# goodmattg/ndivplanning

Hardware: AMD Instinct MI355X
Metric: gan_train_steps_per_sec_traj8_batch64 (higher is better)
Workload: dtype f32; 1 GPU; BASELINE configs[1]: train_gan.py step (D update + G update), codes mode, batch=64 trajectories per GPU, traj_len=8, num_sample=6, noise_dim=2; rows_per_gpu=2688, global_batch=64, parallelism=dp1, hip_graph=True, steps_per_graph_launch=16, repeats=1, gradient_exchange=none

## Files before the change

ndivplanning_amd/csrc/ndp_device.h:

```cpp
#pragma once
#include <hip/hip_runtime.h>
#include <stdint.h>

namespace ndp {

typedef float f32x4 __attribute__((ext_vector_type(4)));
typedef float f32x2 __attribute__((ext_vector_type(2)));
typedef uint32_t u32x4 __attribute__((ext_vector_type(4)));

constexpr int kThreads = 256;
constexpr int kWaves = 4;
constexpr float kLreluSlope = 0.01f;

enum Act { ACT_NONE = 0, ACT_RELU = 1, ACT_LRELU = 2 };

__device__ __forceinline__ int lds_ld(int width) { return width + 4; }

template <int ACT>
__device__ __forceinline__ float act_fwd(float v) {
  if (ACT == ACT_RELU) return v > 0.f ? v : 0.f;
  if (ACT == ACT_LRELU) return v > 0.f ? v : v * kLreluSlope;
  return v;
}

template <int ACT>
__device__ __forceinline__ float act_bwd(float h, float g) {
  if (ACT == ACT_RELU) return h > 0.f ? g : 0.f;
  if (ACT == ACT_LRELU) return h > 0.f ? g : g * kLreluSlope;
  return g;
}

__device__ __forceinline__ void pin_vmem() { __builtin_amdgcn_sched_barrier(0x0786); }
__device__ __forceinline__ void pin_vmem_lds() { __builtin_amdgcn_sched_barrier(0x0606); }

__device__ __forceinline__ f32x4 mfma16(float a, float b, f32x4 c) {
#ifdef NDP_EXP_NOMFMA
  c[0] += a * b;
  return c;
#else
  return __builtin_amdgcn_mfma_f32_16x16x4f32(a, b, c, 0, 0, 0);
#endif
}

__device__ __forceinline__ int fwd_pack_offset(int j, int k, int in, int out) {
  const int per_wave = out >> 2, nt = out >> 6, nit = in >> 4;
  const int wave = j / per_wave, n = (j % per_wave) >> 4, c = j & 15;
  const int t = k >> 4, q = (k & 15) >> 2, e = k & 3;
  return (((wave * nt + n) * nit + t) * 64 + 16 * q + c) * 4 + e;
}
__device__ __forceinline__ int dgrad_pack_offset(int j, int k, int in, int out) {
  const int v_ = in >> 6, nit = out >> 4;
  const int wave = k / (16 * v_), c = (k % (16 * v_)) / v_, v = k % v_;
  const int t = j >> 4, q = (j & 15) >> 2, s = j & 3;
  return (((wave * nit + t) * 64 + 16 * q + c) * 4 + s) * v_ + v;
}

template <class T>
__device__ __forceinline__ T load_kernargs() {
  typedef const __attribute__((address_space(4))) void* kptr_t;
  kptr_t kp = (kptr_t)__builtin_amdgcn_kernarg_segment_ptr();
  constexpr int LAST = (((int)sizeof(T) - 4) / 64) * 64;
  constexpr int O1 = 64 < LAST ? 64 : LAST, O2 = 128 < LAST ? 128 : LAST, O3 = 192 < LAST ? 192 : LAST,
                O4 = 256 < LAST ? 256 : LAST, O5 = 320 < LAST ? 320 : LAST, O6 = 384 < LAST ? 384 : LAST,
                O7 = 448 < LAST ? 448 : LAST;
  static_assert(sizeof(T) <= 576, "argument struct too large for the 8-line prefetch");
  uint32_t t0, t1, t2, t3, t4, t5, t6, t7;
  asm volatile(
      "s_load_dword %0, %8, 0x0\n\ts_load_dword %1, %8, %9\n\ts_load_dword %2, %8, %10\n\t"
      "s_load_dword %3, %8, %11\n\ts_load_dword %4, %8, %12\n\ts_load_dword %5, %8, %13\n\t"
      "s_load_dword %6, %8, %14\n\ts_load_dword %7, %8, %15\n\ts_waitcnt lgkmcnt(0)"
      : "=&s"(t0), "=&s"(t1), "=&s"(t2), "=&s"(t3), "=&s"(t4), "=&s"(t5), "=&s"(t6), "=&s"(t7)
      : "s"(kp), "i"(O1), "i"(O2), "i"(O3), "i"(O4), "i"(O5), "i"(O6), "i"(O7)
      : "memory");
  uint64_t v = (uint64_t)kp;
  asm volatile("" : "+s"(v) : "s"(t0 | t1 | t2 | t3 | t4 | t5 | t6 | t7));
  T out;
  __builtin_memcpy(&out, (kptr_t)v, sizeof(T));
  return out;
}

template <int WALIGN>
__device__ __forceinline__ f32x4 ldg4(const float* p) {
#ifdef NDP_EXP_NOLOAD
  const float v = (float)(reinterpret_cast<uintptr_t>(p) & 1023) * 1e-3f;
  return f32x4{v, v + 1.f, v + 2.f, v + 3.f};
#endif
  if (WALIGN >= 4) {
    return *reinterpret_cast<const f32x4*>(p);
  } else {
    f32x2 lo = *reinterpret_cast<const f32x2*>(p);
    f32x2 hi = *reinterpret_cast<const f32x2*>(p + 2);
    f32x4 r = {lo[0], lo[1], hi[0], hi[1]};
    return r;
  }
}

template <int IN, int OUT, int WALIGN, bool PACKED, int RING = 96>
struct FwdW {
  static constexpr int NT = OUT / 64;
  static constexpr int NIT = IN / 16;
  static constexpr int PF0 = RING / (4 * NT);
  static constexpr int PF = PF0 < NIT ? PF0 : NIT;
  f32x4 ring[PF][NT];
  f32x4 wtail[NT];
  float bias_r[NT];
  const float* wbase;
  int ldw;

  __device__ __forceinline__ f32x4 frag(int n, int t) const {
    if (PACKED) {
      const int wave = threadIdx.x >> 6;
      return ldg4<4>(wbase + (size_t)((wave * NT + n) * NIT + t) * 256);
    }
// ... 306 lines not shown
      g[1] = fmaf(d, w[1], g[1]);
      g[2] = fmaf(d, w[2], g[2]);
      g[3] = fmaf(d, w[3], g[3]);
    }
    f32x4* hp = reinterpret_cast<f32x4*>(H + row * ldh + k);
    f32x4 h = *hp;
    h[0] = act_bwd<ACT>(h[0], g[0]);
    h[1] = act_bwd<ACT>(h[1], g[1]);
    h[2] = act_bwd<ACT>(h[2], g[2]);
    h[3] = act_bwd<ACT>(h[3], g[3]);
    *hp = h;
  }
}

template <int RT, int OUT>
__device__ __forceinline__ void input_dgrad_code(const float* dY, int ldd, const float* __restrict__ W, int ldw,
                                                 float* __restrict__ dX, int64_t ldx, int64_t row0, int64_t m) {
  static_assert(OUT % 16 == 0, "input_dgrad_code shape");
  constexpr int NIT = OUT / 16;
  const int lane = threadIdx.x & 63, wave = threadIdx.x >> 6;
  const int c = lane & 15, q = lane >> 4;
  const float* wp = W + (size_t)(4 * q) * ldw + 64 * wave + c;
  const float* dp = dY + c * ldd + 4 * q;
  f32x4 acc[RT][4];
#pragma unroll
  for (int r = 0; r < RT; ++r)
#pragma unroll
    for (int n = 0; n < 4; ++n) acc[r][n] = f32x4{0.f, 0.f, 0.f, 0.f};
#pragma unroll
  for (int t = 0; t < NIT; ++t) {
    float bv[4][4];
#pragma unroll
    for (int s = 0; s < 4; ++s)
#pragma unroll
      for (int n = 0; n < 4; ++n) bv[s][n] = wp[(size_t)(16 * t + s) * ldw + 16 * n];
    f32x4 av[RT];
#pragma unroll
    for (int r = 0; r < RT; ++r) av[r] = *reinterpret_cast<const f32x4*>(dp + r * 16 * ldd + 16 * t);
#pragma unroll
    for (int s = 0; s < 4; ++s)
#pragma unroll
      for (int r = 0; r < RT; ++r)
#pragma unroll
        for (int n = 0; n < 4; ++n) acc[r][n] = mfma16(av[r][s], bv[s][n], acc[r][n]);
  }
#pragma unroll
  for (int r = 0; r < RT; ++r)
#pragma unroll
    for (int i = 0; i < 4; ++i) {
      const int64_t row = row0 + r * 16 + 4 * q + i;
      if (row < m) {
#pragma unroll
        for (int n = 0; n < 4; ++n) dX[row * ldx + 64 * wave + 16 * n + c] = acc[r][n][i];
      }
    }
}

__device__ __forceinline__ void stg4_wt(float* base, uint32_t off, f32x4 v) {
  const uint64_t ub = reinterpret_cast<uint64_t>(base);
  const uint32_t hi = (uint32_t)__builtin_amdgcn_readfirstlane((int)(ub >> 32));
  const uint32_t lo = (uint32_t)__builtin_amdgcn_readfirstlane((int)(uint32_t)ub);
  const uint64_t sb = ((uint64_t)hi << 32) | (uint64_t)lo;
  const __amdgpu_buffer_rsrc_t rsrc =
      __builtin_amdgcn_make_buffer_rsrc(reinterpret_cast<float*>(sb), 0, 0x7fffffff, 0x00020000);
  __builtin_amdgcn_raw_buffer_store_b128(__builtin_bit_cast(u32x4, v), rsrc, (int)(off * 4u), 0, 16 );
}

template <int RT, int W, bool WT = false>
__device__ __forceinline__ void store_tile(float* __restrict__ dst, size_t gld,
                                           const float* src, int ld) {
  constexpr int R = 16 * RT;
  constexpr int NV = R * W / 4;
#ifdef NDP_EXP_NOSTORE
  if (gld == 0x7fffffff)
#endif
  for (int idx = threadIdx.x; idx < NV; idx += kThreads) {
    const int row = idx / (W / 4), k = 4 * (idx % (W / 4));
    const f32x4 v = *reinterpret_cast<const f32x4*>(src + row * ld + k);
    if constexpr (WT) stg4_wt(dst, (uint32_t)(row * (int)gld + k), v);
    else *reinterpret_cast<f32x4*>(dst + (size_t)row * gld + k) = v;
  }
}

template <int RT, int W>
struct TileRegs {
  static constexpr int NV = 16 * RT * W / 4;
  static constexpr int N = (NV + kThreads - 1) / kThreads;
  f32x4 v[N];
  __device__ __forceinline__ void load(const float* __restrict__ src, size_t gld) {
#pragma unroll
    for (int u = 0; u < N; ++u) {
      int idx = threadIdx.x + u * kThreads;
      idx = idx < NV ? idx : NV - 1;
      const int row = idx / (W / 4), k = 4 * (idx % (W / 4));
      v[u] = ldg4<4>(src + (size_t)row * gld + k);
    }
  }
  __device__ __forceinline__ void store(float* dst, int ld) const {
#pragma unroll
    for (int u = 0; u < N; ++u) {
      const int idx = threadIdx.x + u * kThreads;
      if (idx < NV) {
        const int row = idx / (W / 4), k = 4 * (idx % (W / 4));
        *reinterpret_cast<f32x4*>(dst + row * ld + k) = v[u];
      }
    }
  }
};

template <int RT, int W>
__device__ __forceinline__ void load_tile(float* dst, int ld,
                                          const float* __restrict__ src, size_t gld) {
  constexpr int R = 16 * RT;
  constexpr int NV = R * W / 4;
  for (int idx = threadIdx.x; idx < NV; idx += kThreads) {
    const int row = idx / (W / 4), k = 4 * (idx % (W / 4));
    *reinterpret_cast<f32x4*>(dst + row * ld + k) =
        *reinterpret_cast<const f32x4*>(src + (size_t)row * gld + k);
  }
}

template <int RT>
__device__ __forceinline__ void load_code_tile(float* dst, int ld,
                                               const float* __restrict__ code, int64_t ld_code,
                                               int rep, int64_t row0, int64_t m, bool vec4) {
  constexpr int R = 16 * RT;
  constexpr int NV = R * 64;
  for (int idx = threadIdx.x; idx < NV; idx += kThreads) {
    const int i = idx >> 6, k = 4 * (idx & 63);
    const int64_t row = row0 + i;
    f32x4 v = {0.f, 0.f, 0.f, 0.f};
    if (row < m) {
      const float* p = code + (row / rep) * ld_code + k;
      if (vec4) {
        v = *reinterpret_cast<const f32x4*>(p);
      } else {
        v[0] = p[0]; v[1] = p[1]; v[2] = p[2]; v[3] = p[3];
      }
    }
    *reinterpret_cast<f32x4*>(dst + i * ld + k) = v;
  }
}

__device__ __forceinline__ float wave_sum(float v) {
#pragma unroll
  for (int d = 32; d >= 1; d >>= 1) v += __shfl_xor(v, d, 64);
  return v;
}

__device__ __forceinline__ float block_sum(float v, float* red) {
  v = wave_sum(v);
  if ((threadIdx.x & 63) == 0) red[threadIdx.x >> 6] = v;
  __syncthreads();
  float r = 0.f;
  if (threadIdx.x == 0) {
    const int nw = blockDim.x >> 6;
    for (int w = 0; w < nw; ++w) r += red[w];
  }
  __syncthreads();
  return r;
}

}
```

ndivplanning_amd/csrc/ndp_kernels.hip:

```cpp
#include <hip/hip_runtime.h>
#include <math.h>
#include <stddef.h>
#include <stdint.h>

#include "ndp_device.h"

namespace ndp {

#ifdef NDP_STAMPS
__device__ unsigned long long* g_stamps = nullptr;
__device__ int g_stamp_kernel = 0;
#define NDP_STAMP_ON(id) (g_stamps != nullptr && (g_stamp_kernel == 0 || g_stamp_kernel == (id)))
#define NDP_STAMP_DECL __shared__ unsigned long long stamp_store_[64]; unsigned long long* stamp_lds_ = stamp_store_
#define NDP_STAMP_PTR stamp_lds_
#define NDP_STAMP(i)                                             \
  do {                                                           \
    if (threadIdx.x == 0) {                                      \
      stamp_lds_[2 * (i)] = clock64();                           \
      stamp_lds_[2 * (i) + 1] = wall_clock64();                  \
    }                                                            \
  } while (0)
#define NDP_STAMP_FLUSH(n, id)                                                              \
  do {                                                                                      \
    if (threadIdx.x == 0 && NDP_STAMP_ON(id))                                               \
// ... 435 lines not shown
  GNet net;
  int64_t m;
  const float *h1, *h2, *h3, *h4;
  const float* d_action;
  const float* d_action2;
  float *dy1, *dy2, *dy3, *dy4, *dy5;
};

constexpr int g_bwd_lds_floats() { return 16 * (132 + 68 + 132 + 260 + 4); }

template <bool PK>
__global__ __launch_bounds__(kThreads) void k_g_bwd(GBwdArgs a) {
  constexpr int R = 16;
  extern __shared__ __attribute__((aligned(16))) float smem[];
  float* H1 = smem;
  float* H2 = H1 + R * 132;
  float* H3 = H2 + R * 68;
  float* H4 = H3 + R * 132;
  float* DA = H4 + R * 260;
  const int64_t row0 = (int64_t)blockIdx.x * R;
  const GNet& n = a.net;

  DgW<128, 256, PK> g4;
  g4.preload(PK ? n.pg4 : n.w4, 128);
  load_tile<1, 128>(H1, 132, a.h1 + row0 * 128, 128);
  load_tile<1, 64>(H2, 68, a.h2 + row0 * 64, 64);
  load_tile<1, 128>(H3, 132, a.h3 + row0 * 128, 128);
  load_tile<1, 256>(H4, 260, a.h4 + row0 * 256, 256);
  if (threadIdx.x < R) {
    const int64_t row = row0 + threadIdx.x;
    f32x4 g = {0.f, 0.f, 0.f, 0.f};
    if (row < a.m) {
      g = *reinterpret_cast<const f32x4*>(a.d_action + row * 4);
      if (a.d_action2 != nullptr) g += *reinterpret_cast<const f32x4*>(a.d_action2 + row * 4);
    }
    *reinterpret_cast<f32x4*>(DA + threadIdx.x * 4) = g;
    *reinterpret_cast<f32x4*>(a.dy5 + row * 4) = g;
  }
  __syncthreads();
  layer_dgrad_narrow<1, 256, 4, ACT_RELU>(DA, 4, n.w5, H4, 260);
  __syncthreads();
  DgW<64, 128, PK> g3;
  g3.bind(PK ? n.pg3 : n.w3, 64);
  layer_dgrad_run<1, 128, 256, ACT_RELU, PK>(g4, H4, 260, H3, 132, g3);
  __syncthreads();
  DgW<128, 64, PK> g2;
  g2.bind(PK ? n.pg2 : n.w2, 128);
  layer_dgrad_run<1, 64, 128, ACT_RELU, PK>(g3, H3, 132, H2, 68, g2);
  __syncthreads();
  layer_dgrad_run<1, 128, 64, ACT_RELU, PK>(g2, H2, 68, H1, 132);
  __syncthreads();
  store_tile<1, 128>(a.dy1 + row0 * 128, 128, H1, 132);
  store_tile<1, 64>(a.dy2 + row0 * 64, 64, H2, 68);
  store_tile<1, 128>(a.dy3 + row0 * 128, 128, H3, 132);
  store_tile<1, 256>(a.dy4 + row0 * 256, 256, H4, 260);
}

struct GInGradArgs {
  const float* w1; int ld1, nz;
  const float* dy1;
  float* d_z; int64_t ld_dz;
  int64_t m;
};
__global__ __launch_bounds__(kThreads) void k_g_in_dgrad(GInGradArgs a) {
  constexpr int R = 16;
  __shared__ __attribute__((aligned(16))) float DY[R * 132];
  const int64_t row0 = (int64_t)blockIdx.x * R;
  load_tile<1, 128>(DY, 132, a.dy1 + row0 * 128, 128);
  __syncthreads();
  input_dgrad_code<1, 128>(DY, 132, a.w1, a.ld1, a.d_z, a.ld_dz, row0, a.m);
  const int i = threadIdx.x >> 4, j = threadIdx.x & 15;
  const int64_t row = row0 + i;
  if (j < a.nz && row < a.m) {
    float s = 0.f;
#pragma unroll 8
    for (int o = 0; o < 128; ++o) s = fmaf(DY[i * 132 + o], a.w1[(size_t)o * a.ld1 + CODE + j], s);
    a.d_z[row * a.ld_dz + CODE + j] = s;
  }
}

template <int W, int NP>
__device__ __forceinline__ void store_segment_sums(const float* dY, int ld, float* __restrict__ out,
                                                   int64_t row0, int K, int S, int entries_padded,
                                                   int tile, int ntiles) {
  const int f0 = (int)(row0 / K);
  for (int idx = threadIdx.x; idx < S * W; idx += kThreads) {
    const int sgm = idx / W, col = idx - sgm * W;
    const int64_t lo64 = (int64_t)(f0 + sgm) * K, hi64 = lo64 + K;
    const int lo = (int)(lo64 > row0 ? lo64 - row0 : 0);
    const int hi = (int)(hi64 < row0 + 16 ? hi64 - row0 : 16);
    float acc = 0.f;
    for (int r = lo; r < hi; ++r) {
#pragma unroll
      for (int ps = 0; ps < NP; ++ps) acc += dY[(ps * 16 + r) * ld + col];
    }
    out[((size_t)tile * S + sgm) * W + col] = acc;
  }
  if (tile == ntiles - 1) {
    const int first = ntiles * S;
    for (int idx = threadIdx.x; idx < (entries_padded - first) * W; idx += kThreads) out[(size_t)first * W + idx] = 0.f;
  }
}

struct PhaseAArgs {
  GNet g; DNet d;
  const float* code; int code_rep;
  const float* noise;
  float* noise_out; uint64_t noise_seed; const int32_t* noise_step;
  const float* actions;
  int64_t m, mpad;
  int64_t flat, rpad;
  float inv_m;
  float real_scale;
  float *gh1, *gh2, *gh3, *gh4;
  float* action_hat;
  float *h1, *h2, *h3, *dy1, *dy2, *dy3, *dl, *xa;
  float* loss_partials;
  float* dy1seg; int seg_s, seg_entries;
};

constexpr int kSW5 = 1024 + 8, kSW4 = 256 + 8;
constexpr int phase_a_lds_floats() {
  return 16 * (260 + TAILLD + 132 + 68 + 2) + 16 * 260 + 16 * 4 + 8 + kSW5 + kSW4;
}

template <int OUT, int NR>
__device__ __forceinline__ void code_rows_dot(const float* __restrict__ Wpacked, const float* code, float* part) {
  constexpr int PARTS = kThreads / OUT, SEG = CODE / PARTS;
  const int o = threadIdx.x % OUT, p = threadIdx.x / OUT;
  const float* w = Wpacked + fwd_pack_offset(o, p * SEG, CODE, OUT);
  const float* cr = code + p * SEG;
  float s0[NR], s1[NR];
#pragma unroll
  for (int j = 0; j < NR; ++j) s0[j] = s1[j] = 0.f;
#pragma unroll 2
  for (int t = 0; t < SEG / 16; ++t) {
#pragma unroll
    for (int q = 0; q < 4; ++q) {
      const f32x4 wv = *reinterpret_cast<const f32x4*>(w + t * 256 + q * 64);
#pragma unroll
      for (int j = 0; j < NR; ++j) {
        const f32x4 cv = *reinterpret_cast<const f32x4*>(cr + j * 260 + 16 * t + 4 * q);
        s0[j] = fmaf(wv[0], cv[0], s0[j]); s1[j] = fmaf(wv[1], cv[1], s1[j]);
        s0[j] = fmaf(wv[2], cv[2], s0[j]); s1[j] = fmaf(wv[3], cv[3], s1[j]);
      }
    }
  }
#pragma unroll
  for (int j = 0; j < NR; ++j) part[(j * PARTS + p) * OUT + o] = s0[j] + s1[j];
}
template <int NR>
__device__ __forceinline__ void load_code_rows(float* XC, const float* __restrict__ code, int64_t f0, int64_t nflat) {
  const int j = threadIdx.x >> 6, c4 = threadIdx.x & 63;
  if (j < NR) {
    f32x4 v = {0.f, 0.f, 0.f, 0.f};
    if (f0 + j < nflat) v = *reinterpret_cast<const f32x4*>(code + (size_t)(f0 + j) * CODE + 4 * c4);
    *reinterpret_cast<f32x4*>(XC + j * 260 + 4 * c4) = v;
  }
}
template <int OUT, int ACT, int NR>
__device__ __forceinline__ void fc1_from_code_rows(const float* part, const float* __restrict__ bias,
                                                   const float* __restrict__ Wt, int ldw, int ntail,
                                                   const float* XT, float* Y, int ldy, int rem0, int K) {
  constexpr int PARTS = kThreads / OUT, RSTEP = kThreads / OUT;
  const int o = threadIdx.x % OUT, r0 = threadIdx.x / OUT;
  float wt[16];
#pragma unroll
  for (int j = 0; j < 16; ++j) wt[j] = j < ntail ? Wt[(size_t)o * ldw + j] : 0.f;
  float base[NR];
#pragma unroll
  for (int j = 0; j < NR; ++j) {
    base[j] = bias[o];
#pragma unroll
    for (int p = 0; p < PARTS; ++p) base[j] += part[(j * PARTS + p) * OUT + o];
  }
  for (int r = r0; r < 16; r += RSTEP) {
    float s = base[0];
    if (NR > 1) {
      const int x = rem0 + r;
      const int idx = (x >= K) + (x >= 2 * K) + (x >= 3 * K);
#pragma unroll
      for (int j = 1; j < NR; ++j) s = idx >= j ? base[j] : s;
    }
#pragma unroll
    for (int j = 0; j < 16; ++j)
      if (j < ntail) s = fmaf(XT[r * TAILLD + j], wt[j], s);
    Y[r * ldy + o] = act_fwd<ACT>(s);
  }
}

constexpr bool kWtTilesCu1 = true;
constexpr bool kWtTilesLargeM = false;
constexpr bool kWtSlabs = true;
constexpr bool kWtSlabsWide = false;
constexpr bool wt_tiles(int RG) { return RG >= 96 ? kWtTilesCu1 : kWtTilesLargeM; }

template <bool PK, int RG, int NR>
__device__ __forceinline__ void phase_a_d_part(const PhaseAArgs& a, bool real, int tile, int ntiles,
                                               FwdW<256, 64, 4, PK, RG>& dw1, FwdW<64, 128, 4, PK, RG>& dw2, const float* cpd,
                                               float* XC, float* XT, float* B1,
                                               float* B2, float* L, float* DL, const float* W4S,
                                               unsigned long long* stamp_lds_) {
  constexpr int R = 16;
  constexpr bool WT = wt_tiles(RG);
  const DNet& d = a.d;
  (void)stamp_lds_;
  const int64_t row0 = (int64_t)tile * R;
  const int64_t nvalid = real ? a.flat : a.m;
  const int64_t g0 = (real ? 0 : a.rpad) + row0;
  NDP_STAMP(10);
  if (NR > 0) {
    fc1_from_code_rows<64, ACT_LRELU, (NR > 0 ? NR : 1)>(cpd, d.b1, d.w1, 260, ADIM, XT, B2, 68,
                                                         (int)(row0 % a.code_rep), a.code_rep);
  } else {
    dw2.bind(PK ? d.pf2 : d.w2, 64, d.b2, nullptr, 0);
    layer_fwd_run<1, 256, 64, ACT_LRELU, 4, PK>(dw1, XC, 260, B2, 68, XT, TAILLD, dw2);
  }
  NDP_STAMP(11);
  __syncthreads();
  NDP_STAMP(3);
  FwdW<128, 256, 4, PK, RG> dw3;
  dw3.bind(PK ? d.pf3 : d.w3, 128, d.b3, nullptr, 0);
  layer_fwd_run<1, 64, 128, ACT_LRELU, 4, PK>(dw2, B2, 68, B1, 132, nullptr, 0, dw3);
  __syncthreads();
  DgW<128, 256, PK, RG> dg3;
  dg3.bind(PK ? d.pg3 : d.w3, 128);
  layer_fwd_run<1, 128, 256, ACT_LRELU, 4, PK>(dw3, B1, 132, XC, 260, nullptr, 0, dg3);
  __syncthreads();
  NDP_STAMP(4);
  layer_fwd_narrow<1, 256, 1>(XC, 260, W4S, W4S + 256, L, 1);
  __syncthreads();
  float lsum = 0.f;
  if (threadIdx.x < R) {
    const int64_t row = row0 + threadIdx.x;
    const float target = real ? 1.f : 0.f;
    const float weight = real ? a.real_scale : 1.f;
    const float x = L[threadIdx.x];
    float dl = 0.f;
    if (row < nvalid) {
      lsum = weight * (fmaxf(x, 0.f) - x * target + log1pf(expf(-fabsf(x))));
      dl = weight * ((1.f / (1.f + expf(-x)) - target) * a.inv_m);
    }
    DL[threadIdx.x] = dl;
    a.dl[g0 + threadIdx.x] = dl;
  }
  if (threadIdx.x < 64) {
    const float tot = wave_sum(lsum);
    if (threadIdx.x == 0) a.loss_partials[blockIdx.x] = tot;
  }
  NDP_STAMP(5);
  store_tile<1, 64, WT>(a.h1 + g0 * 64, 64, B2, 68);
  store_tile<1, 128, WT>(a.h2 + g0 * 128, 128, B1, 132);
  store_tile<1, 256, WT>(a.h3 + g0 * 256, 256, XC, 260);
  if (threadIdx.x < R)
    if constexpr (WT) stg4_wt(a.xa + g0 * 4, 4 * threadIdx.x, *reinterpret_cast<const f32x4*>(XT + threadIdx.x * TAILLD));
    else *reinterpret_cast<f32x4*>(a.xa + (g0 + threadIdx.x) * 4) = *reinterpret_cast<const f32x4*>(XT + threadIdx.x * TAILLD);
  __syncthreads();
  NDP_STAMP(6);
  layer_dgrad_narrow<1, 256, 1, ACT_LRELU>(DL, 1, W4S, XC, 260);
  __syncthreads();
  DgW<64, 128, PK, RG> dg2;
  dg2.bind(PK ? d.pg2 : d.w2, 64);
  layer_dgrad_run<1, 128, 256, ACT_LRELU, PK>(dg3, XC, 260, B1, 132, dg2);
  __syncthreads();
  NDP_STAMP(7);
  layer_dgrad_run<1, 64, 128, ACT_LRELU, PK>(dg2, B1, 132, B2, 68);
  __syncthreads();
  if (real) store_tile<1, 64, WT>(a.dy1seg + ((size_t)a.seg_entries + row0) * 64, 64, B2, 68);
  else store_segment_sums<64, 1>(B2, 68, a.dy1seg, row0, a.code_rep, a.seg_s, a.seg_entries, tile, ntiles);
  store_tile<1, 64, WT>(a.dy1 + g0 * 64, 64, B2, 68);
  store_tile<1, 128, WT>(a.dy2 + g0 * 128, 128, B1, 132);
  store_tile<1, 256, WT>(a.dy3 + g0 * 256, 256, XC, 260);
}

constexpr int kPhaseASmallRing = 24;
template <bool PK, int RG, int NR>
__global__ __launch_bounds__(kThreads, (RG >= 96 ? 1 : 3)) void k_phase_a(PhaseAArgs a_segment) {
  constexpr bool DD = NR > 0;
  constexpr int NRR = NR > 0 ? NR : 1;
  constexpr bool WT = wt_tiles(RG);
  const PhaseAArgs a = RG >= 96 ? load_kernargs<PhaseAArgs>() : a_segment;
  constexpr int R = 16;
  extern __shared__ __attribute__((aligned(16))) float smem[];
  float* XC = smem;
  float* XT = XC + R * 260;
  float* B1 = XT + R * TAILLD;
  float* B2 = B1 + R * 132;
  float* B3 = B2 + R * 68;
  float* A = B3 + R * 260;
  float* L = A + R * 4;
  float* DL = L + R;
  float* red = DL + R;
  float* W5S = red + 8;
  float* W4S = W5S + kSW5;
  const int ntiles = (int)(a.mpad / R);
  const bool real = (int)blockIdx.x >= ntiles;
  const GNet& g = a.g;
  const DNet& d = a.d;
  NDP_STAMP_DECL;
  NDP_STAMP(0);

  FwdW<256, 64, 4, PK, RG> dw1;
  FwdW<64, 128, 4, PK, RG> dw2;
  if (!real) {
    const int tile = (int)blockIdx.x;
    const int64_t row0 = (int64_t)tile * R;
    FwdW<256, 128, 2, PK, RG> gw1;
    FwdW<128, 64, 4, PK, RG> gw2;
    f32x4 ct[R * 64 / kThreads];
    if (DD) {
      load_code_rows<NRR>(XC, a.code, (int64_t)((uint32_t)row0 / (uint32_t)a.code_rep), a.flat);
    } else {
#pragma unroll
      for (int u = 0; u < R * 64 / kThreads; ++u) {
        const int idx = threadIdx.x + u * kThreads;
        const int i = idx >> 6, k = 4 * (idx & 63);
        const int64_t row = row0 + i;
        const bool ok = row < a.m;
        const f32x4 v = *reinterpret_cast<const f32x4*>(a.code + (size_t)((uint32_t)(ok ? row : 0) / (uint32_t)a.code_rep) * CODE + k);
        ct[u] = ok ? v : f32x4{0.f, 0.f, 0.f, 0.f};
      }
    }
    const f32x4 w5r = *reinterpret_cast<const f32x4*>(g.w5 + 4 * threadIdx.x);
    const float b5r = g.b5[threadIdx.x & 3], w4r = d.w4[threadIdx.x], b4r = d.b4[0];
    float nv = 0.f;
    {
      static_assert(R * TAILLD == kThreads, "one noise element per thread");
      const int i = threadIdx.x / TAILLD, t = threadIdx.x % TAILLD;
      const int64_t row = row0 + i;
      if (row < a.m && t < g.nz) {
        if (a.noise_out != nullptr) {
          nv = philox_uniform((uint64_t)(row * g.nz + t), a.noise_seed, (uint32_t)*a.noise_step);
          a.noise_out[row * g.nz + t] = nv;
        } else {
          nv = a.noise[row * g.nz + t];
        }
      }
    }
    pin_vmem();
    if (DD) gw2.preload(PK ? g.pf2 : g.w2, 128, g.b2, nullptr, 0);
    else gw1.preload(PK ? g.pf1 : g.w1, g.ld1, g.b1, g.w1 + CODE, g.nz);
    NDP_STAMP(24);
    if (!DD) {
#pragma unroll
      for (int u = 0; u < R * 64 / kThreads; ++u) {
        const int idx = threadIdx.x + u * kThreads;
        *reinterpret_cast<f32x4*>(XC + (idx >> 6) * 260 + 4 * (idx & 63)) = ct[u];
      }
    }
    NDP_STAMP(25);
    XT[threadIdx.x] = nv;
    *reinterpret_cast<f32x4*>(W5S + 4 * threadIdx.x) = w5r;
    if (threadIdx.x < 4) W5S[1024 + threadIdx.x] = b5r;
    W4S[threadIdx.x] = w4r;
    if (threadIdx.x == 0) W4S[256] = b4r;
// ... 130 lines not shown
  const DNet& d = a.d;
  NDP_STAMP_DECL;
  NDP_STAMP(0);

  FwdW<256, 64, 4, PK, RG> dw1;
  FwdW<64, 128, 4, PK, RG> dw2;
  f32x4 ct[R * 64 / kThreads];
  float av = 0.f;
  {
    if (DD) {
      load_code_rows<NRR>(XC, a.code, row0 / a.code_rep, (a.m + a.code_rep - 1) / a.code_rep);
    } else {
#pragma unroll
      for (int u = 0; u < R * 64 / kThreads; ++u) {
        const int idx = threadIdx.x + u * kThreads;
        const int i = idx >> 6, k = 4 * (idx & 63);
        const int64_t row = row0 + i;
        const bool ok = row < a.m;
        const f32x4 v = *reinterpret_cast<const f32x4*>(a.code + ((ok ? row : 0) / a.code_rep) * CODE + k);
        ct[u] = ok ? v : f32x4{0.f, 0.f, 0.f, 0.f};
      }
    }
    const int i = threadIdx.x / TAILLD, t = threadIdx.x % TAILLD;
    const int64_t row = row0 + i;
    if (row < a.m && t < ADIM) av = a.action_hat[row * ADIM + t];
  }
  const float w1a = d.w1[(threadIdx.x >> 2) * 260 + (threadIdx.x & 3)], w4r = d.w4[threadIdx.x], b4r = d.b4[0];
  const f32x4 w5r = *reinterpret_cast<const f32x4*>(g.w5 + 4 * threadIdx.x);
  pin_vmem();
  if (DD) dw2.preload(PK ? d.pf2 : d.w2, 64, d.b2, nullptr, 0);
  else dw1.preload(PK ? d.pf1 : d.w1 + ADIM, 260, d.b1, d.w1, ADIM);
  if (!DD) {
#pragma unroll
    for (int u = 0; u < R * 64 / kThreads; ++u) {
      const int idx = threadIdx.x + u * kThreads;
      *reinterpret_cast<f32x4*>(XC + (idx >> 6) * 260 + 4 * (idx & 63)) = ct[u];
    }
  }
  XT[threadIdx.x] = av;
  TileRegs<1, 128> t1;
  TileRegs<1, 256> t4;
  TileRegs<1, 128> t3;
  TileRegs<1, 64> t2;
  W1A[threadIdx.x] = w1a;
  W4S[threadIdx.x] = w4r;
  if (threadIdx.x == 0) W4S[256] = b4r;
  *reinterpret_cast<f32x4*>(W5S + 4 * threadIdx.x) = w5r;
  if (PRE) {
    t1.load(a.gh1 + row0 * 128, 128);
    t4.load(a.gh4 + row0 * 256, 256);
    t3.load(a.gh3 + row0 * 128, 128);
    t2.load(a.gh2 + row0 * 64, 64);
    pin_vmem();
  } else {
    load_tile<1, 128>(H1, 132, a.gh1 + row0 * 128, 128);
  }
  __syncthreads();
  NDP_STAMP(1);
  if (DD) {
    code_rows_dot<64, NRR>(d.pf1, XC, XC + NRR * 260);
    __syncthreads();
    fc1_from_code_rows<64, ACT_LRELU, NRR>(XC + NRR * 260, d.b1, d.w1, 260, ADIM, XT, B2, 68,
                                           (int)(row0 % a.code_rep), a.code_rep);
  } else {
    dw2.bind(PK ? d.pf2 : d.w2, 64, d.b2, nullptr, 0);
    layer_fwd_run<1, 256, 64, ACT_LRELU, 4, PK>(dw1, XC, 260, B2, 68, XT, TAILLD, dw2);
  }
  if (PRE) {
    t1.store(H1, 132);
    t4.store(G4, 260);
    t3.store(G3, 132);
    t2.store(G2, 68);
  }
  __syncthreads();
  FwdW<128, 256, 4, PK, RG> dw3;
  dw3.bind(PK ? d.pf3 : d.w3, 128, d.b3, nullptr, 0);
  layer_fwd_run<1, 64, 128, ACT_LRELU, 4, PK>(dw2, B2, 68, B1, 132, nullptr, 0, dw3);
  __syncthreads();
  DgW<128, 256, PK, RG> dg3;
  dg3.bind(PK ? d.pg3 : d.w3, 128);
  layer_fwd_run<1, 128, 256, ACT_LRELU, 4, PK>(dw3, B1, 132, XC, 260, nullptr, 0, dg3);
  __syncthreads();
  NDP_STAMP(2);
  layer_fwd_narrow<1, 256, 1>(XC, 260, W4S, W4S + 256, L, 1);
  __syncthreads();
  float lsum = 0.f;
  if (threadIdx.x < R) {
    const int64_t row = row0 + threadIdx.x;
    const float x = L[threadIdx.x];
    float dl = 0.f;
    if (row < a.m) {
      lsum = fmaxf(x, 0.f) - x + log1pf(expf(-fabsf(x)));
      dl = (1.f / (1.f + expf(-x)) - 1.f) * a.inv_m;
    }
    DL[threadIdx.x] = dl;
  }
  if (threadIdx.x < 64) {
    const float tot = wave_sum(lsum);
    if (threadIdx.x == 0) a.loss_partials[blockIdx.x] = tot;
  }
  __syncthreads();
  NDP_STAMP(3);
  layer_dgrad_narrow<1, 256, 1, ACT_LRELU>(DL, 1, W4S, XC, 260);
  __syncthreads();
  DgW<64, 128, PK, RG> dg2;
  dg2.bind(PK ? d.pg2 : d.w2, 64);
  layer_dgrad_run<1, 128, 256, ACT_LRELU, PK>(dg3, XC, 260, B1, 132, dg2);
  __syncthreads();
  DgW<128, 256, PK, RG> gg4;
  gg4.bind(PK ? g.pg4 : g.w4, 128);
  layer_dgrad_run<1, 64, 128, ACT_LRELU, PK>(dg2, B1, 132, B2, 68, gg4);
  __syncthreads();
  NDP_STAMP(4);
  {
    const int i = threadIdx.x >> 4, j = (threadIdx.x >> 2) & 3, part = threadIdx.x & 3;
    const int64_t row = row0 + i;
    const float ng = (part == 0 && row < a.m && a.nd_grad != nullptr) ? a.nd_grad[row * ADIM + j] : 0.f;
    float s = 0.f;
#pragma unroll
    for (int o = 16 * part; o < 16 * part + 16; ++o) s = fmaf(B2[i * 68 + o], W1A[o * 4 + j], s);
    s += __shfl_xor(s, 1, 64);
    s += __shfl_xor(s, 2, 64);
    if (part == 0) {
      s = row < a.m ? s + ng : 0.f;
      DA[i * ADIM + j] = s;
      a.dy5[row * ADIM + j] = s;
    }
  }
  __syncthreads();
  NDP_STAMP(5);

  if (!PRE) {
    load_tile<1, 256>(G4, 260, a.gh4 + row0 * 256, 256);
    load_tile<1, 128>(G3, 132, a.gh3 + row0 * 128, 128);
    load_tile<1, 64>(G2, 68, a.gh2 + row0 * 64, 64);
    __syncthreads();
  }
  NDP_STAMP(6);
  layer_dgrad_narrow<1, 256, 4, ACT_RELU>(DA, 4, W5S, G4, 260);
  __syncthreads();
  NDP_STAMP(7);
  DgW<64, 128, PK, RG> gg3;
  gg3.bind(PK ? g.pg3 : g.w3, 64);
  layer_dgrad_run<1, 128, 256, ACT_RELU, PK>(gg4, G4, 260, G3, 132, gg3);
  __syncthreads();
  NDP_STAMP(8);
  DgW<128, 64, PK, RG> gg2;
  gg2.bind(PK ? g.pg2 : g.w2, 128);
  store_tile<1, 256, WT>(a.dy4 + row0 * 256, 256, G4, 260);
  layer_dgrad_run<1, 64, 128, ACT_RELU, PK>(gg3, G3, 132, G2, 68, gg2);
  __syncthreads();
  NDP_STAMP(9);
  store_tile<1, 128, WT>(a.dy3 + row0 * 128, 128, G3, 132);
  layer_dgrad_run<1, 128, 64, ACT_RELU, PK>(gg2, G2, 68, H1, 132);
  __syncthreads();
  NDP_STAMP(10);
  store_tile<1, 64, WT>(a.dy2 + row0 * 64, 64, G2, 68);
  store_tile<1, 128, WT>(a.dy1 + row0 * 128, 128, H1, 132);
  store_segment_sums<128, 1>(H1, 132, a.dy1seg, row0, a.code_rep, a.seg_s, a.seg_entries, (int)blockIdx.x, (int)gridDim.x);
  NDP_STAMP(11);
  NDP_STAMP_FLUSH(12, 6);
}

__device__ __forceinline__ void adam_advance(int32_t* state, float lr, float b1, float b2) {
  const int32_t t = state[0] + 1;
  state[0] = t;
  const double bc1 = 1.0 - pow((double)b1, (double)t);
  const double bc2 = 1.0 - pow((double)b2, (double)t);
  reinterpret_cast<float*>(state)[1] = (float)((double)lr / bc1);
  reinterpret_cast<float*>(state)[2] = (float)sqrt(bc2);
}

enum { WG_FULL = 0, WG_SKINNY_B = 1, WG_SKINNY_A = 2, WG_WIDE = 3 };
constexpr int kWgradPrefetch = 8;

struct WgradJob {
  const float* A;
  const float* B;
  int lda, ldb;
  int a_cols, b_cols;
  int b_rowmod, b_rowdiv, b_rowmax;
  int b_vec;
  int dst_off, dst_ld;
  int bias_off;
  int kind;
  int rows, seg, seg_s, seg_k;
  int seg_wrap;
  int nchunks;
};
constexpr int kMaxJobs = 28;
struct WgradHead {
  int njobs;
  int nwide;
  int wide_chunks;
  int rows;
  float* slabs;
  int64_t slab_stride;
  int32_t* bump;
  float lr, beta1, beta2;
  int nchunks;
  NdivArgs nd;
};
struct WgradArgs : WgradHead {
  WgradJob job[kMaxJobs];
  int net_is_g;
  int nreg, reg_begin[4], reg_end[4];
  int wide_begin, wide_end;
// ... 520 lines not shown
```

Before: 13120 steps/s.

## Defer per-row loss scaling through dgrad and overlap BCE loss with next layer

The final 256->1 discriminator layer now computes its output and writes the unscaled activation-derivative mask in a single pass, instead of waiting for the loss gradient. The per-row loss scale is applied later, when the dgrad results are stored or consumed, which works because the backward pass is linear in that scalar. The BCE loss math runs as a job interleaved into the next dgrad layer's weight preload slices, which removes two block barriers and a narrow dgrad pass. In exchange there is extra per-element scaling at store time, and intermediate dgrad buffers now hold unscaled values, so every consumer of them must apply the scale correctly.

Result: no change. 13240 steps/s, median of 6 (+0.9%).

```diff
diff --git a/ndivplanning_amd/csrc/ndp_device.h b/ndivplanning_amd/csrc/ndp_device.h
--- a/ndivplanning_amd/csrc/ndp_device.h
+++ b/ndivplanning_amd/csrc/ndp_device.h
@@ -29,6 +29,8 @@
   if (ACT == ACT_LRELU) return h > 0.f ? g : g * kLreluSlope;
   return g;
 }
+
+__device__ __forceinline__ float row_scaled(float dl, float u) { return dl == 0.f ? 0.f : dl * u; }
 
 __device__ __forceinline__ void pin_vmem() { __builtin_amdgcn_sched_barrier(0x0786); }
 __device__ __forceinline__ void pin_vmem_lds() { __builtin_amdgcn_sched_barrier(0x0606); }
@@ -501,6 +503,76 @@
   }
 }
 
+template <int IN, int ACT, bool WT>
+__device__ __forceinline__ void narrow1_fwd_unit(float* H, int ldh, const float* __restrict__ W,
+                                                 const float* __restrict__ bias, float* Y, float* __restrict__ gh) {
+  constexpr int PARTS = kThreads / 16;
+  constexpr int NV = IN / 4 / PARTS;
+  static_assert(IN % (4 * PARTS) == 0, "narrow1_fwd_unit shape");
+  const int row = threadIdx.x / PARTS, part = threadIdx.x % PARTS;
+  float sum = 0.f;
+#pragma unroll
+  for (int m = 0; m < NV; ++m) {
+    const int k = 4 * (part + PARTS * m);
+    f32x4* hp = reinterpret_cast<f32x4*>(H + row * ldh + k);
+    const f32x4 x = *hp;
+    const f32x4 w = *reinterpret_cast<const f32x4*>(W + k);
+    sum = fmaf(x[0], w[0], sum);
+    sum = fmaf(x[1], w[1], sum);
+    sum = fmaf(x[2], w[2], sum);
+    sum = fmaf(x[3], w[3], sum);
+    if (gh != nullptr) {
+      if constexpr (WT) stg4_wt(gh, (uint32_t)(row * IN + k), x);
+      else *reinterpret_cast<f32x4*>(gh + (size_t)row * IN + k) = x;
+    }
+    f32x4 u;
+#pragma unroll
+    for (int e = 0; e < 4; ++e) u[e] = act_bwd<ACT>(x[e], w[e]);
+    *hp = u;
+  }
+#pragma unroll
+  for (int d = PARTS / 2; d >= 1; d >>= 1) sum += __shfl_xor(sum, d, 64);
+  if (part == 0) Y[row] = sum + bias[0];
+}
+
+template <int RT, int W, bool WT>
+__device__ __forceinline__ void store_tile_rows(float* __restrict__ dst, size_t gld, const float* src, int ld,
+                                                const float* dl) {
+  constexpr int NV = 16 * RT * W / 4;
+  for (int idx = threadIdx.x; idx < NV; idx += kThreads) {
+    const int row = idx / (W / 4), k = 4 * (idx % (W / 4));
+    f32x4 v = *reinterpret_cast<const f32x4*>(src + row * ld + k);
+    const float s = dl[row];
+#pragma unroll
+    for (int e = 0; e < 4; ++e) v[e] = row_scaled(s, v[e]);
+    if constexpr (WT) stg4_wt(dst, (uint32_t)(row * (int)gld + k), v);
+    else *reinterpret_cast<f32x4*>(dst + (size_t)row * gld + k) = v;
+  }
+}
+
+template <class NEXT, class JOB>
+struct WithJob {
+  NEXT& next;
+  JOB& job;
+  __device__ __forceinline__ void preload_slice(int t, int nslices) {
+    next.preload_slice(t, nslices);
+    job(t);
+  }
+};
+__device__ __forceinline__ void job_fence() { __builtin_amdgcn_sched_barrier(0); }
+
+template <int CTRL>
+__device__ __forceinline__ float dpp_row(float x) {
+  return __builtin_bit_cast(float, __builtin_amdgcn_update_dpp(0, __builtin_bit_cast(int, x), CTRL, 0xf, 0xf, true));
+}
+__device__ __forceinline__ float row16_sum_lane0(float v) {
+  v += dpp_row<0x128>(v);
+  v += dpp_row<0x124>(v);
+  v += dpp_row<0x4E>(v);
+  v += dpp_row<0xB1>(v);
+  return v;
+}
+
 template <int RT, int W>
 struct TileRegs {
   static constexpr int NV = 16 * RT * W / 4;
diff --git a/ndivplanning_amd/csrc/ndp_kernels.hip b/ndivplanning_amd/csrc/ndp_kernels.hip
--- a/ndivplanning_amd/csrc/ndp_kernels.hip
+++ b/ndivplanning_amd/csrc/ndp_kernels.hip
@@ -541,7 +541,7 @@
 template <int W, int NP>
 __device__ __forceinline__ void store_segment_sums(const float* dY, int ld, float* __restrict__ out,
                                                    int64_t row0, int K, int S, int entries_padded,
-                                                   int tile, int ntiles) {
+                                                   int tile, int ntiles, const float* dl = nullptr) {
   const int f0 = (int)(row0 / K);
   for (int idx = threadIdx.x; idx < S * W; idx += kThreads) {
     const int sgm = idx / W, col = idx - sgm * W;
@@ -551,7 +551,7 @@
     float acc = 0.f;
     for (int r = lo; r < hi; ++r) {
 #pragma unroll
-      for (int ps = 0; ps < NP; ++ps) acc += dY[(ps * 16 + r) * ld + col];
+      for (int ps = 0; ps < NP; ++ps) acc += dl != nullptr ? row_scaled(dl[r], dY[(ps * 16 + r) * ld + col]) : dY[(ps * 16 + r) * ld + col];
     }
     out[((size_t)tile * S + sgm) * W + col] = acc;
   }
@@ -653,6 +653,8 @@
 constexpr bool kWtSlabs = true;
 constexpr bool kWtSlabsWide = false;
 constexpr bool wt_tiles(int RG) { return RG >= 96 ? kWtTilesCu1 : kWtTilesLargeM; }
+
+constexpr int kLossAt = 1, kLossCommit = 10;
 
 template <bool PK, int RG, int NR>
 __device__ __forceinline__ void phase_a_d_part(const PhaseAArgs& a, bool real, int tile, int ntiles,
@@ -687,49 +689,50 @@
   layer_fwd_run<1, 128, 256, ACT_LRELU, 4, PK>(dw3, B1, 132, XC, 260, nullptr, 0, dg3);
   __syncthreads();
   NDP_STAMP(4);
-  layer_fwd_narrow<1, 256, 1>(XC, 260, W4S, W4S + 256, L, 1);
-  __syncthreads();
-  float lsum = 0.f;
-  if (threadIdx.x < R) {
-    const int64_t row = row0 + threadIdx.x;
-    const float target = real ? 1.f : 0.f;
-    const float weight = real ? a.real_scale : 1.f;
-    const float x = L[threadIdx.x];
-    float dl = 0.f;
-    if (row < nvalid) {
-      lsum = weight * (fmaxf(x, 0.f) - x * target + log1pf(expf(-fabsf(x))));
-      dl = weight * ((1.f / (1.f + expf(-x)) - target) * a.inv_m);
-    }
-    DL[threadIdx.x] = dl;
-    a.dl[g0 + threadIdx.x] = dl;
-  }
-  if (threadIdx.x < 64) {
-    const float tot = wave_sum(lsum);
-    if (threadIdx.x == 0) a.loss_partials[blockIdx.x] = tot;
-  }
+  store_tile<1, 128, WT>(a.h2 + g0 * 128, 128, B1, 132);
+  narrow1_fwd_unit<256, ACT_LRELU, WT>(XC, 260, W4S, W4S + 256, L, a.h3 + g0 * 256);
+  __syncthreads();
   NDP_STAMP(5);
   store_tile<1, 64, WT>(a.h1 + g0 * 64, 64, B2, 68);
-  store_tile<1, 128, WT>(a.h2 + g0 * 128, 128, B1, 132);
-  store_tile<1, 256, WT>(a.h3 + g0 * 256, 256, XC, 260);
   if (threadIdx.x < R)
     if constexpr (WT) stg4_wt(a.xa + g0 * 4, 4 * threadIdx.x, *reinterpret_cast<const f32x4*>(XT + threadIdx.x * TAILLD));
     else *reinterpret_cast<f32x4*>(a.xa + (g0 + threadIdx.x) * 4) = *reinterpret_cast<const f32x4*>(XT + threadIdx.x * TAILLD);
-  __syncthreads();
   NDP_STAMP(6);
-  layer_dgrad_narrow<1, 256, 1, ACT_LRELU>(DL, 1, W4S, XC, 260);
-  __syncthreads();
+  float dl = 0.f, tot = 0.f;
+  auto loss = [&](int t) {
+    if (t == kLossAt) {
+      const int64_t row = row0 + (threadIdx.x & 15);
+      const float target = real ? 1.f : 0.f;
+      const float weight = real ? a.real_scale : 1.f;
+      const float x = L[threadIdx.x & 15];
+      const float bce = weight * (fmaxf(x, 0.f) - x * target + log1pf(expf(-fabsf(x))));
+      const float sg = weight * ((1.f / (1.f + expf(-x)) - target) * a.inv_m);
+      const bool mine = threadIdx.x < R && row < nvalid;
+      dl = mine ? sg : 0.f;
+      tot = row16_sum_lane0(mine ? bce : 0.f);
+    }
+    if (t == kLossCommit) {
+      job_fence();
+      if (threadIdx.x < R) {
+        DL[threadIdx.x] = dl;
+        a.dl[g0 + threadIdx.x] = dl;
+        if (threadIdx.x == 0) a.loss_partials[blockIdx.x] = tot;
+      }
+    }
+  };
   DgW<64, 128, PK, RG> dg2;
   dg2.bind(PK ? d.pg2 : d.w2, 64);
-  layer_dgrad_run<1, 128, 256, ACT_LRELU, PK>(dg3, XC, 260, B1, 132, dg2);
+  WithJob<decltype(dg2), decltype(loss)> dg2_loss{dg2, loss};
+  layer_dgrad_run<1, 128, 256, ACT_LRELU, PK>(dg3, XC, 260, B1, 132, dg2_loss);
   __syncthreads();
   NDP_STAMP(7);
   layer_dgrad_run<1, 64, 128, ACT_LRELU, PK>(dg2, B1, 132, B2, 68);
   __syncthreads();
-  if (real) store_tile<1, 64, WT>(a.dy1seg + ((size_t)a.seg_entries + row0) * 64, 64, B2, 68);
-  else store_segment_sums<64, 1>(B2, 68, a.dy1seg, row0, a.code_rep, a.seg_s, a.seg_entries, tile, ntiles);
-  store_tile<1, 64, WT>(a.dy1 + g0 * 64, 64, B2, 68);
-  store_tile<1, 128, WT>(a.dy2 + g0 * 128, 128, B1, 132);
-  store_tile<1, 256, WT>(a.dy3 + g0 * 256, 256, XC, 260);
+  if (real) store_tile_rows<1, 64, WT>(a.dy1seg + ((size_t)a.seg_entries + row0) * 64, 64, B2, 68, DL);
+  else store_segment_sums<64, 1>(B2, 68, a.dy1seg, row0, a.code_rep, a.seg_s, a.seg_entries, tile, ntiles, DL);
+  store_tile_rows<1, 64, WT>(a.dy1 + g0 * 64, 64, B2, 68, DL);
+  store_tile_rows<1, 128, WT>(a.dy2 + g0 * 128, 128, B1, 132, DL);
+  store_tile_rows<1, 256, WT>(a.dy3 + g0 * 256, 256, XC, 260, DL);
 }
 
 constexpr int kPhaseASmallRing = 24;
@@ -1026,30 +1029,32 @@
   layer_fwd_run<1, 128, 256, ACT_LRELU, 4, PK>(dw3, B1, 132, XC, 260, nullptr, 0, dg3);
   __syncthreads();
   NDP_STAMP(2);
-  layer_fwd_narrow<1, 256, 1>(XC, 260, W4S, W4S + 256, L, 1);
-  __syncthreads();
-  float lsum = 0.f;
-  if (threadIdx.x < R) {
-    const int64_t row = row0 + threadIdx.x;
-    const float x = L[threadIdx.x];
-    float dl = 0.f;
-    if (row < a.m) {
-      lsum = fmaxf(x, 0.f) - x + log1pf(expf(-fabsf(x)));
-      dl = (1.f / (1.f + expf(-x)) - 1.f) * a.inv_m;
-    }
-    DL[threadIdx.x] = dl;
-  }
-  if (threadIdx.x < 64) {
-    const float tot = wave_sum(lsum);
-    if (threadIdx.x == 0) a.loss_partials[blockIdx.x] = tot;
-  }
+  narrow1_fwd_unit<256, ACT_LRELU, false>(XC, 260, W4S, W4S + 256, L, nullptr);
   __syncthreads();
   NDP_STAMP(3);
-  layer_dgrad_narrow<1, 256, 1, ACT_LRELU>(DL, 1, W4S, XC, 260);
-  __syncthreads();
+  float dl = 0.f, tot = 0.f;
+  auto loss = [&](int t) {
+    if (t == kLossAt) {
+      const int64_t row = row0 + (threadIdx.x & 15);
+      const float x = L[threadIdx.x & 15];
+      const float bce = fmaxf(x, 0.f) - x + log1pf(expf(-fabsf(x)));
+      const float sg = (1.f / (1.f + expf(-x)) - 1.f) * a.inv_m;
+      const bool mine = threadIdx.x < R && row < a.m;
+      dl = mine ? sg : 0.f;
+      tot = row16_sum_lane0(mine ? bce : 0.f);
+    }
+    if (t == kLossCommit) {
+      job_fence();
+      if (threadIdx.x < R) {
+        DL[threadIdx.x] = dl;
+        if (threadIdx.x == 0) a.loss_partials[blockIdx.x] = tot;
+      }
+    }
+  };
   DgW<64, 128, PK, RG> dg2;
   dg2.bind(PK ? d.pg2 : d.w2, 64);
-  layer_dgrad_run<1, 128, 256, ACT_LRELU, PK>(dg3, XC, 260, B1, 132, dg2);
+  WithJob<decltype(dg2), decltype(loss)> dg2_loss{dg2, loss};
+  layer_dgrad_run<1, 128, 256, ACT_LRELU, PK>(dg3, XC, 260, B1, 132, dg2_loss);
   __syncthreads();
   DgW<128, 256, PK, RG> gg4;
   gg4.bind(PK ? g.pg4 : g.w4, 128);
@@ -1066,7 +1071,7 @@
     s += __shfl_xor(s, 1, 64);
     s += __shfl_xor(s, 2, 64);
     if (part == 0) {
-      s = row < a.m ? s + ng : 0.f;
+      s = row < a.m ? row_scaled(DL[i], s) + ng : 0.f;
       DA[i * ADIM + j] = s;
       a.dy5[row * ADIM + j] = s;
     }
```
